# IvanIZ/BenchPush

Hardware: AMD Instinct MI355X
Metric: env-steps/sec at N=4096 envs (ship-ice-v0), 1/2/4/8 MI355X (higher is better)
Workload: dtype f64

## Files before the change

benchpush_amd/build.py:

```python
import os
import subprocess

_HERE = os.path.dirname(os.path.abspath(__file__))
CSRC = os.path.join(_HERE, "csrc")
LIB_PATH = os.path.join(_HERE, "libbenchpush_hip.so")
SOURCES = ["bp_capi.hip"]


def _headers():
    import glob
    return sorted(glob.glob(os.path.join(CSRC, "*.hpp"))) + [os.path.join(_HERE, "..", "include", "benchpush_amd.h")]

HIPCC_FLAGS = ["--offload-arch=gfx950", "-O3", "-ffp-contract=off", "-fno-fast-math", "-fPIC", "-shared", "-std=c++17",
               "-Wno-unused-value"]


def needs_build():
    if not os.path.exists(LIB_PATH):
        return True
    t = os.path.getmtime(LIB_PATH)
    for p in [os.path.join(CSRC, f) for f in SOURCES] + _headers():
        if os.path.exists(p) and os.path.getmtime(p) > t:
            return True
    return False


def build_hip(force=False, verbose=False):
    if not force and not needs_build():
        return LIB_PATH
    hipcc = os.environ.get("HIPCC", "/opt/rocm/bin/hipcc")
    if not os.path.exists(hipcc):
        hipcc = "hipcc"
    cmd = [hipcc] + HIPCC_FLAGS + ["-o", LIB_PATH] + [os.path.join(CSRC, s) for s in SOURCES]
    if verbose:
        print(" ".join(cmd))
    subprocess.check_call(cmd, cwd=CSRC)
    return LIB_PATH


DBG_LIB_PATH = os.path.join(_HERE, "libbenchpush_hip_dbgpaths.so")


def build_debug_paths(force=False, verbose=False):
    if not force and os.path.exists(DBG_LIB_PATH):
        t = os.path.getmtime(DBG_LIB_PATH)
        if all(os.path.getmtime(p) <= t for p in [os.path.join(CSRC, f) for f in SOURCES] + _headers() if os.path.exists(p)):
            return DBG_LIB_PATH
    hipcc = os.environ.get("HIPCC", "/opt/rocm/bin/hipcc")
    if not os.path.exists(hipcc):
        hipcc = "hipcc"
    cmd = [hipcc] + HIPCC_FLAGS + ["-DBP_DEBUG_PATHS=1", "-o", DBG_LIB_PATH] + [os.path.join(CSRC, s) for s in SOURCES]
    if verbose:
        print(" ".join(cmd))
    subprocess.check_call(cmd, cwd=CSRC)
    return DBG_LIB_PATH


PROF_LIB_PATH = os.path.join(_HERE, "libbenchpush_hip_prof.so")


def build_prof(force=False, verbose=False):
    if not force and os.path.exists(PROF_LIB_PATH):
        t = os.path.getmtime(PROF_LIB_PATH)
        if all(os.path.getmtime(p) <= t for p in [os.path.join(CSRC, f) for f in SOURCES] + _headers() if os.path.exists(p)):
            return PROF_LIB_PATH
    hipcc = os.environ.get("HIPCC", "/opt/rocm/bin/hipcc")
    if not os.path.exists(hipcc):
        hipcc = "hipcc"
    cmd = [hipcc] + HIPCC_FLAGS + ["-DBP_PROF=1", "-o", PROF_LIB_PATH] + [os.path.join(CSRC, s) for s in SOURCES]
    if verbose:
        print(" ".join(cmd))
    subprocess.check_call(cmd, cwd=CSRC)
    return PROF_LIB_PATH


if __name__ == "__main__":
    print(build_hip(force=True, verbose=True))
    print(build_debug_paths(force=True, verbose=True))
    print(build_prof(force=True, verbose=True))
```

benchpush_amd/csrc/bp_physics.hpp:

```cpp
#pragma once
#include "bp_device.hpp"
#include <type_traits>

#ifdef BP_PROF
#define PROF_DECL unsigned long long _pt = __builtin_amdgcn_s_memtime();
#define PROF_ACC(slot) { unsigned long long _n = __builtin_amdgcn_s_memtime(); if (lane_id() == 0) L.prof[slot] += _n - _pt; _pt = _n; }
#define PROF_CNT(slot, v) { const unsigned long long _v = (unsigned long long)(v); if (lane_id() == 0) L.prof[slot] += _v; }
#define PROF_MAX(slot, v) { const unsigned long long _v = (unsigned long long)(v); if (lane_id() == 0 && _v > L.prof[slot]) L.prof[slot] = _v; }
#define PROF_PARAM , unsigned long long &_pt
#define PROF_ARG , _pt
#else
#define PROF_DECL
#define PROF_ACC(slot)
#define PROF_CNT(slot, v)
#define PROF_MAX(slot, v)
#define PROF_PARAM
#define PROF_ARG
#endif


#define BP_UNLIKELY(x) __builtin_expect(!!(x), 0)
#define BP_UNLIKELY2(x) __builtin_expect(!!(x), 0)
#ifdef BP_DEBUG_PATHS
#define BP_DBGP(bit) ((P.dbg_paths & (bit)) != 0)
#define BP_TRACE_ON(D) ((D).dbg != nullptr)
#else
#define BP_DBGP(bit) false
#define BP_TRACE_ON(D) false
#endif
#ifndef BP_BOUND_GROUPS
#define BP_BOUND_GROUPS 3
#endif
#ifndef BP_MANIFOLD_LANES
#define BP_MANIFOLD_LANES 2
#endif
#include "bp_contact.hpp"

struct EnvCtx {
    int nb;
    const int *nv;
    const d2 *lv, *ln;
    const double4 *mass;
    const double4 *prop;
    const int *kind;
    d2 *pxy, *rot, *wv, *wn, *pv;
    double *ang;
    double4 *bb, *fat;
    unsigned short *adj;
    unsigned char *adjn;
    unsigned long long *hint;
};

template <typename T> __device__ __forceinline__ T &gE(T *const base, const int idx) { return *(T *)((char *)base + (size_t)((unsigned)idx * (unsigned)sizeof(T))); }

struct LdsCtx {
    d2 *sv, *sw, *sb;
    d2 *ag;
    d2 *sp;
    unsigned char *slot_of;
    unsigned *mvs;
    unsigned short *owner;
    unsigned short *colmask;
    d2 *tf;
    unsigned short *mv;
    unsigned *mvo;
    unsigned short *sbody;
    unsigned char *rf;
// ... 323 lines not shown
        const bool hitQ = (xh & 1) != 0;
        const unsigned h = sd ? ((unsigned)(xh >> 1) << 8) | (unsigned)eia : ((unsigned)eia << 8) | (unsigned)(xh >> 1);
        const bool any = hit || hitQ, two = hit && hitQ;
        PROF_CNT(54, (unsigned long long)__popcll(ballot(sd == 0 && hit && !hitQ)) | ((unsigned long long)__popcll(ballot(sd == 0 && !hit && hitQ)) << 32))
        PROF_CNT(55, __popcll(ballot(sd == 0 && two)))
        PROF_ACC(10)
        const bool flagonly = (cw & (1u << 19)) != 0;
        if (ballot(any && flagonly)) S.wall_flag = 1;
        const bool del = any && !flagonly;
        const unsigned long long dm = ballot(del && sd == 0);
        const int drank = popc_below(dm, lane & ~1);
        const int ndel = __popcll(dm);
        const unsigned keyv = (e.x << 16) | (e.x >> 16);
        lds_sync();
        for (int dbase = 0; dbase < ndel; dbase += BP_MBOX) {
            if (del && drank >= dbase && drank < dbase + BP_MBOX) {
                d2 *mb = L.mbox + (drank - dbase) * 6;
                if (sd == 0) {
                    mb[0] = n;
                    if (hit) { mb[1] = p1; mb[2] = p2; mb[5].x = __hiloint2double((int)h, two ? 2 : 1); }
                } else {
                    if (!hitQ) { mb[1] = p1; mb[2] = p2; mb[5].x = __hiloint2double((int)h, 1); }
                    mb[3] = two ? p1 : mk2(0, 0); mb[4] = two ? p2 : mk2(0, 0);
                    mb[5].y = __hiloint2double(two ? (int)h : 0, 0);
                }
            }
            lds_sync();
            arbiters_take(E, L, A, S, dm, dbase, keyv, now);
            lds_sync();
        }
    }
}

template <int KIND, bool DAMP = false>
__device__ __forceinline__ void substep(const DevParams &P, const EnvCtx &E, const LdsCtx &L, ArbReg &A, SubState &S,
                                        const double dt, const int ship_rules)
{
    const int lane = lane_id();
    constexpr int VL = (KIND == BP_ENV_BOX) ? 4 : (KIND == BP_ENV_MAZE) ? 8 : BP_MAXV;
    constexpr bool ML2 = (BP_MANIFOLD_LANES == 2) && KIND != BP_ENV_BOX;
    if (KIND == BP_ENV_BOX) { S.nev = 0; S.evmask = 0ull; }
    S.stamp += 1u;
    const unsigned now = S.stamp;
    const double prev_dt = S.curr_dt;
    S.curr_dt = dt;
    if (A.key != ARB_FREE_KEY && A.stamp == now - 1u) A.state = ARB_NORMAL;
    PROF_DECL
    PROF_CNT(16, S.nmv)

    for (int k0 = 0; k0 < S.nmv; k0 += 64) {
        const int k = k0 + lane;
        double rad = 0.0;
        double4 fatb; fatb.x = fatb.y = -BP_INF; fatb.z = fatb.w = BP_INF;
        if (k < S.nmv) {
            const int i = L.mv[k];
            const int sl = L.slot_of[i];
            d2 v = mk2(0.0, 0.0), w2 = mk2(0.0, 0.0), vb = mk2(0.0, 0.0);
            if (sl != 255) { v = L.sv[sl]; w2 = L.sw[sl]; vb = L.sb[sl]; }
            d2 p = gE(E.pxy, i);
            if (sl != 255) p = L.sp[sl];
            const double a = gE(E.ang, i);
            d2 r = gE(E.rot, i);
            const double4 ms = gE(E.mass, i);
            rad = gE(E.prop, i).x;
            fatb = gE(E.fat, i);
            L.rf[lane] = (unsigned char)gE(E.nv, i);
            p.x = p.x + (v.x + vb.x) * dt;
            p.y = p.y + (v.y + vb.y) * dt;
            const double a2 = a + (w2.x + w2.y) * dt;
            if (a2 != a) { double sn, cs; bp_sincos(a2, sn, cs); r = mk2(cs, sn); }
            gE(E.pxy, i) = p; gE(E.ang, i) = a2; gE(E.rot, i) = r;
            if (i == 0) { L.ag[0] = mk2(a2, 0.0); L.ag[1] = r; }
            if (sl != 255) { L.sb[sl] = mk2(0.0, 0.0); L.sw[sl].y = 0.0; L.sp[sl] = p; }
// ... 40 lines not shown
            nbb.x = key_f64(bbk[lane * 4 + 0]) - rad; nbb.y = key_f64(bbk[lane * 4 + 2]) - rad;
            nbb.z = key_f64(bbk[lane * 4 + 1]) + rad; nbb.w = key_f64(bbk[lane * 4 + 3]) + rad;
            gE(E.bb, i) = nbb;
            leftfat = !(nbb.x >= fatb.x && nbb.y >= fatb.y && nbb.z <= fatb.z && nbb.w <= fatb.w);
        }
        PROF_ACC(0)
        unsigned long long rm = ballot(leftfat);
        if (BP_UNLIKELY(rm != 0)) { S.cc_ok = 0; __syncthreads(); }
        while (BP_UNLIKELY(rm != 0)) {
            const int kk = __ffsll((long long)rm) - 1;
            rm &= rm - 1;
            refresh_body(P, E, L.mv[k0 + kk], S.err);
            PROF_CNT(17, 1)
        }
        PROF_ACC(1)
    }
    __syncthreads();
    PROF_ACC(35)

    int kmax = S.cc_kmax;
    if (!S.cc_ok) {
        kmax = 0;
        for (int k0 = 0; k0 < S.nmv; k0 += 64) {
            const int k = k0 + lane;
            const int cnt = (k < S.nmv) ? (int)gE(E.adjn, L.mv[k]) : 0;
            int m = 0;
            for (int bit = 16; bit >= 1; bit >>= 1) { if (ballot(cnt >= (m | bit))) m |= bit; }
            kmax = max(kmax, m);
        }
        S.cc_kmax = kmax;
    }
    const int ncand_slots = S.nmv * kmax;
    for (int base = 0; base < ncand_slots; base += 64) {
        int i, j, s, nA_h, nB_h;
        bool valid, flagonly;
        unsigned long long hw;
        const bool cached = S.cc_ok && base == 0 && !BP_DBGP(1);
        if (cached) {
            const unsigned long long c = L.cc[lane];
            hw = L.cc_hw[lane];
            static_assert(2 * BP_CC_IDX_BITS == 28, "cc word layout: i | j << BP_CC_IDX_BITS | slot << 28 ...");
            i = (int)(c & ((1u << BP_CC_IDX_BITS) - 1u)); j = (int)((c >> BP_CC_IDX_BITS) & ((1u << BP_CC_IDX_BITS) - 1u)); s = (int)((c >> 28) & 31u);
            nA_h = (int)((c >> 33) & 31u); nB_h = (int)((c >> 38) & 31u);
            valid = ((c >> 43) & 1u) != 0; flagonly = ((c >> 44) & 1u) != 0;
        } else {
            const int idx = base + lane;
            const int k = idx / kmax;
            s = idx - k * kmax;
            const bool inlist = k < S.nmv;
            i = inlist ? (int)L.mv[k] : 0;
            const int sc = min(s, BP_KADJ - 1);
            const int adjn_i = gE(E.adjn, i);
            j = gE(E.adj, i * BP_KADJ + sc) < E.nb ? (int)gE(E.adj, i * BP_KADJ + sc) : 0;
            hw = gE(E.hint, i * BP_KADJ + sc);
            valid = inlist && (s < adjn_i);
            if (valid && L.mvs[j] == now && j < i) valid = false;
            const int ki = gE(E.kind, i), kj = gE(E.kind, j);
            const double mi = gE(E.mass, i).x, mj = gE(E.mass, j).x;
            nA_h = gE(E.nv, min(i, j)); nB_h = gE(E.nv, max(i, j));
            flagonly = false;
            if (valid) {
                if (kind_group(ki) != 0 && kind_group(ki) == kind_group(kj)) valid = false;
                else if (mi == 0.0 && mj == 0.0) {
                    const int ci = kind_ctype(ki), cj = kind_ctype(kj);
                    flagonly = (ci == 1 && cj == 3) || (ci == 3 && cj == 1);
                    valid = flagonly;
                }
            }
            s = min(s, 31);
            if (base == 0) {
                L.cc[lane] = (unsigned long long)(unsigned)i | ((unsigned long long)(unsigned)j << BP_CC_IDX_BITS) | ((unsigned long long)(unsigned)s << 28) |
                             ((unsigned long long)(unsigned)nA_h << 33) | ((unsigned long long)(unsigned)nB_h << 38) |
                             ((unsigned long long)(valid ? 1u : 0u) << 43) | ((unsigned long long)(flagonly ? 1u : 0u) << 44);
                L.cc_hw[lane] = hw;
            }
        }
        const int sc = min(s, BP_KADJ - 1);
        const int sa = min(i, j), sb = max(i, j);
        const double4 bbi = gE(E.bb, i);
        const double4 bbj = gE(E.bb, j);
        const double radA = gE(E.prop, sa).x, radB = gE(E.prop, sb).x;
        const double rsum = radA + radB;
        const int hA = HW_PLANE_A(hw) < BP_MAXV ? HW_PLANE_A(hw) : 0, hB = HW_PLANE_B(hw) < BP_MAXV ? HW_PLANE_B(hw) : 0;
        const int cnA = HW_NV_A(hw), cnB = HW_NV_B(hw);
        const int jA0 = HW_VERT_A(hw) < BP_MAXV ? HW_VERT_A(hw) : 0, jB0 = HW_VERT_B(hw) < BP_MAXV ? HW_VERT_B(hw) : 0;
        const int jAm = (jA0 == 0) ? max(min(cnB, BP_MAXV) - 1, 0) : jA0 - 1, jAp = (jA0 + 1 >= cnB) ? 0 : jA0 + 1;
        const int jBm = (jB0 == 0) ? max(min(cnA, BP_MAXV) - 1, 0) : jB0 - 1, jBp = (jB0 + 1 >= cnA) ? 0 : jB0 + 1;
        const d2 fnA = gE(E.wn, sa * BP_MAXV + hA), fpA = gE(E.wv, sa * BP_MAXV + hA);
        const d2 fnB = gE(E.wn, sb * BP_MAXV + hB), fpB = gE(E.wv, sb * BP_MAXV + hB);
        const d2 vAm = gE(E.wv, sb * BP_MAXV + jAm), vA0 = gE(E.wv, sb * BP_MAXV + jA0), vAp = gE(E.wv, sb * BP_MAXV + jAp);
        const d2 vBm = gE(E.wv, sa * BP_MAXV + jBm), vB0 = gE(E.wv, sa * BP_MAXV + jB0), vBp = gE(E.wv, sa * BP_MAXV + jBp);
        if (valid) valid = bb_overlap(bbi, bbj);
        PROF_ACC(27)
        PROF_CNT(24, 1)
        PROF_CNT(36, __popcll(ballot(valid)))
        if (ballot(valid) == 0) { PROF_ACC(2) continue; }
        const bool evA = valid && (hw & HW_HAS_A) && ((hw & HW_BOTH) || !(hw & HW_PRIM_B));
        const bool evB = valid && (hw & HW_HAS_B) && ((hw & HW_BOTH) || (hw & HW_PRIM_B));
        double sepAc = -BP_INF, sepBc = -BP_INF;
        int jAc = jA0, jBc = jB0;
        const double cA = vdot(fnA, fpA), cB = vdot(fnB, fpB);
        bool qryA = evA, qryB = evB;
        {
            const double dm = vdot(fnA, vAm), d0 = vdot(fnA, vA0), dp = vdot(fnA, vAp);
            if (evA && cnB == nB_h && cnB >= 2 && d0 + BP_SUPPORT_MARGIN <= dm && d0 + BP_SUPPORT_MARGIN <= dp && !BP_DBGP(4)) { sepAc = (d0 - cA) + 0.0; qryA = false; }
        }
        {
            const double dm = vdot(fnB, vBm), d0 = vdot(fnB, vB0), dp = vdot(fnB, vBp);
            if (evB && cnA == nA_h && cnA >= 2 && d0 + BP_SUPPORT_MARGIN <= dm && d0 + BP_SUPPORT_MARGIN <= dp && !BP_DBGP(4)) { sepBc = (d0 - cB) + 0.0; qryB = false; }
        }
        {
            const unsigned long long mqA = ballot(qryA), mqB = ballot(qryB);
            const int nqA = __popcll(mqA), nq1 = nqA + __popcll(mqB);
            PROF_CNT(37, nq1)
            if (BP_UNLIKELY(nq1)) {
                const int slA = popc_below(mqA, lane), slB = nqA + popc_below(mqB, lane);
                for (int q0 = 0; q0 < nq1; q0 += BP_QCAP) {
                    const bool inA = qryA && slA >= q0 && slA < q0 + BP_QCAP, inB = qryB && slB >= q0 && slB < q0 + BP_QCAP;
                    if (inA) { L.q_dir[slA - q0] = fnA; L.q_meta[slA - q0] = (unsigned)sb | ((unsigned)nB_h << 16); }
                    if (inB) { L.q_dir[slB - q0] = fnB; L.q_meta[slB - q0] = (unsigned)sa | ((unsigned)nA_h << 16); }
                    lds_sync();
                    support_queries<VL>(E, L, min(nq1 - q0, BP_QCAP));
                    lds_sync();
                    if (inA) { sepAc = (L.r_val[slA - q0] - cA) + 0.0; jAc = (int)L.r_idx[slA - q0]; }
                    if (inB) { sepBc = (L.r_val[slB - q0] - cB) + 0.0; jBc = (int)L.r_idx[slB - q0]; }
                    lds_sync();
                }
            }
        }
        if (valid && (sepAc > rsum || sepBc > rsum)) {
            valid = false;
            if (hw & HW_BOTH) {
                const unsigned long long nh = (hw & ~(HW_BOTH | HW_PRIM_B)) | ((sepAc > rsum) ? 0ull : HW_PRIM_B);
                gE(E.hint, i * BP_KADJ + s) = nh;
                if (base == 0) L.cc_hw[lane] = nh;
            }
        }
        const unsigned long long cm = ballot(valid);
        PROF_ACC(28)
        PROF_CNT(18, __popcll(cm))
        if (cm == 0) continue;
        PROF_CNT(25, 1)
        const int nc = __popcll(cm);
        const int myr = popc_below(cm, lane);
        const int nA_l = valid ? nA_h : 0, nB_l = valid ? nB_h : 0;
        if (valid) {
            uint4 pa;
            pa.x = (unsigned)sa | ((unsigned)sb << 16);
            pa.y = (unsigned)nA_l | (evA ? 0x80u : 0u) | ((unsigned)nB_l << 8) | ((unsigned)hA << 16) | ((unsigned)jAc << 24);
            pa.z = (unsigned)sb | ((unsigned)sa << 16);
            pa.w = (unsigned)nB_l | (evB ? 0x80u : 0u) | ((unsigned)nA_l << 8) | ((unsigned)hB << 16) | ((unsigned)jBc << 24);
            L.pt_a[myr] = pa;
            L.pt_thr[myr] = mk2(sepAc, sepBc);
            L.res_smA[myr] = evA ? f64_key(sepAc) : 0ull; L.res_iA[myr] = evA ? ((unsigned)hA << 8) | (unsigned)jAc : 0xFFFFFFFFu;
            L.res_smB[myr] = evB ? f64_key(sepBc) : 0ull; L.res_iB[myr] = evB ? ((unsigned)hB << 8) | (unsigned)jBc : 0xFFFFFFFFu;
            static_assert(BP_CC_IDX_BITS + 5 <= 19 && BP_KADJ <= 32, "candidate lane's word: i | slot << BP_CC_IDX_BITS | flagonly << 19 | lane << 20");
            if (ML2) L.res_jA[myr] = (unsigned)i | ((unsigned)s << BP_CC_IDX_BITS) | (flagonly ? 1u << 19 : 0u) | ((unsigned)lane << 20);
        }
        lds_sync();
        {
            int nq = 0, g0 = 0;
            const uint2 *const pts = (const uint2 *)L.pt_a;
            const double *const pts_thr = (const double *)L.pt_thr;
            auto round_addr = [&](const uint2 e, int &pbody, int &qbody, int &np, int &nqv, int &hX, bool &evX, int &jc, int &jm, int &jp) {
                pbody = (int)(e.x & 0xFFFFu); qbody = (int)(e.x >> 16);
                np = (int)(e.y & 0x7Fu); evX = (e.y & 0x80u) != 0; nqv = (int)((e.y >> 8) & 0xFFu);
                hX = (int)((e.y >> 16) & 0xFFu); jc = (int)(e.y >> 24);
                jm = (jc == 0) ? max(nqv, 1) - 1 : jc - 1; jp = (jc + 1 >= nqv) ? 0 : jc + 1;
            };
            int rr_start = nc;
            {
                constexpr int GW = (BP_BOUND_GROUPS == 3 && KIND != BP_ENV_BOX) ? BP_MAXV + 1 : 32, IPR = 64 / GW;
                static_assert(GW >= BP_MAXV && IPR * GW <= 64, "a lane group holds every plane of a side");
                const int g = lane / GW, f = lane - g * GW;
                const int ipr = BP_DBGP(16) ? 1 : IPR;
                bool fits = !BP_DBGP(2);
                for (int r0 = 0; r0 < nc && fits; r0 += ipr) {
                    const bool on0 = g < ipr && 2 * r0 + g < 2 * nc, on1 = g < ipr && 2 * r0 + ipr + g < 2 * nc;
                    const int ta = on0 ? 2 * r0 + g : 2 * r0, tb = on1 ? 2 * r0 + ipr + g : 2 * r0;
                    const uint2 e0 = pts[ta], e1 = pts[tb];
                    const double th0 = pts_thr[ta], th1 = pts_thr[tb];
                    int pb0, qb0, np0, nqv0, hX0, jc0, jm0, jp0, pb1, qb1, np1, nqv1, hX1, jc1, jm1, jp1; bool ev0, ev1;
                    round_addr(e0, pb0, qb0, np0, nqv0, hX0, ev0, jc0, jm0, jp0);
                    round_addr(e1, pb1, qb1, np1, nqv1, hX1, ev1, jc1, jm1, jp1);
                    const int fc0 = (f < np0) ? f : 0, fc1 = (f < np1) ? f : 0;
                    const d2 fn0 = gE(E.wn, pb0 * BP_MAXV + fc0), fp0 = gE(E.wv, pb0 * BP_MAXV + fc0), vb0 = gE(E.wv, qb0 * BP_MAXV + jc0), vm0 = gE(E.wv, qb0 * BP_MAXV + jm0), vp0 = gE(E.wv, qb0 * BP_MAXV + jp0);
                    const d2 fn1 = gE(E.wn, pb1 * BP_MAXV + fc1), fp1 = gE(E.wv, pb1 * BP_MAXV + fc1), vb1 = gE(E.wv, qb1 * BP_MAXV + jc1), vm1 = gE(E.wv, qb1 * BP_MAXV + jm1), vp1 = gE(E.wv, qb1 * BP_MAXV + jp1);
                    {
                        const bool pv = on0 && (f < np0) && !(ev0 && f == hX0);
                        const double c = vdot(fn0, fp0);
// ... 18 lines not shown
                        if (surv && sl < BP_QCAP) {
                            L.q_dir[sl] = fn1; L.q_meta[sl] = (unsigned)qb1 | ((unsigned)nqv1 << 16);
                            L.q_aux[sl] = (unsigned)(tb >> 1) | ((unsigned)(tb & 1) << 8) | ((unsigned)f << 16);
                            L.q_c[sl] = c;
                        }
                        nq += __popcll(sm);
                    }
                    PROF_CNT(49, 1)
                    fits = nq <= BP_QCAP;
                }
                if (!fits) { nq = 0; rr_start = 0; }
                lds_sync();
            }
            const int side = lane >> 5, f = lane & 31;
            for (int rr = rr_start; rr <= nc; rr++) {
                if (nq > 0 && (rr == nc || nq + 64 > BP_QCAP)) {
                    PROF_ACC(29)
                    support_queries<VL>(E, L, nq);
                    lds_sync();
                    PROF_CNT(26, 1)
                    PROF_CNT(38, nq)
                    for (int s0 = 0; s0 < nq; s0 += 64) {
                        const int sl = s0 + lane;
                        if (sl < nq) {
                            const unsigned aux = L.q_aux[sl];
                            const int r = (int)(aux & 0xFFu);
                            const double sp = (L.r_val[sl] - L.q_c[sl]) + 0.0;
                            const unsigned long long key = f64_key(sp);
                            L.q_c[sl] = __builtin_bit_cast(double, key);
                            atomicMax((aux & 0x100u) ? &L.res_smB[r] : &L.res_smA[r], key);
                        }
                    }
                    lds_sync();
                    if (valid && myr >= g0 && myr < rr) {
                        if (evA && f64_key(sepAc) != L.res_smA[myr]) L.res_iA[myr] = 0xFFFFFFFFu;
                        if (evB && f64_key(sepBc) != L.res_smB[myr]) L.res_iB[myr] = 0xFFFFFFFFu;
                    }
                    lds_sync();
                    for (int s0 = 0; s0 < nq; s0 += 64) {
                        const int sl = s0 + lane;
                        if (sl < nq) {
                            const unsigned aux = L.q_aux[sl];
                            const int r = (int)(aux & 0xFFu);
                            const unsigned long long key = __builtin_bit_cast(unsigned long long, L.q_c[sl]);
                            if (key == ((aux & 0x100u) ? L.res_smB[r] : L.res_smA[r])) atomicMin((aux & 0x100u) ? &L.res_iB[r] : &L.res_iA[r], ((aux >> 16) << 8) | L.r_idx[sl]);
                        }
                    }
                    lds_sync();
                    nq = 0; g0 = rr;
                    PROF_ACC(30)
                }
                if (rr == nc) break;
                const uint2 e = pts[2 * rr + side];
                const double th = pts_thr[2 * rr + side];
                int pbody, qbody, np, nqv, hX, jc, jm, jp; bool evX;
                round_addr(e, pbody, qbody, np, nqv, hX, evX, jc, jm, jp);
                const bool pv = (f < np) && !(evX && f == hX);
                const int fc = (f < np) ? f : 0;
                const d2 fn = gE(E.wn, pbody * BP_MAXV + fc), fp = gE(E.wv, pbody * BP_MAXV + fc);
                const d2 vb = gE(E.wv, qbody * BP_MAXV + jc), vm = gE(E.wv, qbody * BP_MAXV + jm), vp = gE(E.wv, qbody * BP_MAXV + jp);
                const double c = vdot(fn, fp);
                const double bound = (fmin(vdot(fn, vb), fmin(vdot(fn, vm), vdot(fn, vp))) - c) + 0.0;
                const bool surv = pv && (!evX || bound >= th);
                const unsigned long long sm = ballot(surv);
                if (surv) {
                    const int sl = nq + popc_below(sm, lane);
                    L.q_dir[sl] = fn; L.q_meta[sl] = (unsigned)qbody | ((unsigned)nqv << 16);
// ... 426 lines not shown
                if (AB) {
                    const d2 vb1 = vadd(vba, vmul(vperp(r1), wa2.y));
                    const d2 vb2 = vadd(vbb, vmul(vperp(r2), wb2.y));
                    const double vbn = vdot(vsub(vb2, vb1), n);
                    const double jbn = (bias - vbn) * nMass;
                    jBias = fmax(jbnOld + jbn, 0.0);
                }
                const double jn = -(bounce + vrn) * nMass;
                const double jnOld = c ? A.jn1 : A.jn0;
                const double jnAcc = fmax(jnOld + jn, 0.0);
                const double jtMax = A.u * jnAcc;
                const double jt = -vrt * tMass;
                const double jtOld = c ? A.jt1 : A.jt0;
                const double jtAcc = fclampd(jtOld + jt, -jtMax, jtMax);
                if (c) { jBias1 = jBias; A.jn1 = jnAcc; A.jt1 = jtAcc; }
                else   { jBias0 = jBias; A.jn0 = jnAcc; A.jt0 = jtAcc; }
                if (AB) {
                    const double djb = jBias - jbnOld;
                    chg += __builtin_fabs(djb);
                    const d2 jb = vmul(n, djb);
                    const d2 jbneg = vneg(jb);
                    vba = vadd(vba, vmul(jbneg, A.ma));
                    wa2.y += A.ia * vcross(r1, jbneg);
                    vbb = vadd(vbb, vmul(jb, A.mb));
                    wb2.y += A.ib * vcross(r2, jb);
                }
                const double djn = jnAcc - jnOld, djt = jtAcc - jtOld;
                chg += __builtin_fabs(djn); chg += __builtin_fabs(djt);
                const d2 j = vrotate(n, mk2(djn, djt));
                apply_contact_impulses(A, c, va, wa2.x, vb, wb2.x, j);
            }
        }
    };
    if (!AB && KIND != BP_ENV_BOX && (lvlmask & (lvlmask - 1u)) == 0u && lvlmask != 0u) {
        d2 va = mk2(0.0, 0.0), vb = va, wa2 = va, wb2 = va, vba = va, vbb = va;
        if (solve) gather(va, vb, wa2, wb2, vba, vbb);
        bool nz = false;
        if (solve && A.ma == 0.0) nz = is_negzero(va.x) || is_negzero(va.y) || is_negzero(wa2.x) || (AB && (is_negzero(wa2.y) || is_negzero(vba.x) || is_negzero(vba.y)));
        if (solve && A.mb == 0.0) nz = nz || is_negzero(vb.x) || is_negzero(vb.y) || is_negzero(wb2.x) || (AB && (is_negzero(wb2.y) || is_negzero(vbb.x) || is_negzero(vbb.y)));
        if (!ballot(nz)) {
            for (int it = 0; it < P.iterations; it++) {
                PROF_CNT(42, 1)
                PROF_CNT(43, 1)
                double chg = 0.0;
                if (solve) contacts(va, vb, wa2, wb2, vba, vbb, chg);
                if (BP_UNLIKELY2(!ballot(solve && chg != 0.0))) break;
            }
            if (solve) scatter(va, vb, wa2, wb2, vba, vbb);
            lds_sync();
            return;
        }
    }
    for (int it = 0; it < P.iterations; it++) {
        PROF_CNT(42, 1)
        double chg = 0.0;
        for (unsigned lm = lvlmask; lm; lm &= lm - 1u) {
            const int lvl = __ffs((int)lm) - 1;
            PROF_CNT(43, 1)
            PROF_CNT(44, ballot(solve && A.level == lvl && A.count > 1) ? 1 : 0)
            if (solve && A.level == lvl) {
                d2 va, vb, wa2, wb2, vba, vbb;
                gather(va, vb, wa2, wb2, vba, vbb);
                contacts(va, vb, wa2, wb2, vba, vbb, chg);
                scatter(va, vb, wa2, wb2, vba, vbb);
            }
            lds_sync();
        }
        if (BP_UNLIKELY2(!ballot(solve && chg != 0.0))) break;
    }
    };
    if (any_bias && !mirrored) iterate(std::true_type{}); else iterate(std::false_type{});
    PROF_ACC(8)
    {
        const bool shiparb = active && ba == 0;
        const unsigned long long sm = ballot(shiparb);
        S.ship_post = (unsigned)__popcll(sm);
        S.ship_contacts = (unsigned)__popcll(sm) + (unsigned)__popcll(ballot(shiparb && A.count > 1));
        if (sm) {
            S.n_post += (unsigned)__popcll(sm);
            S.n_contact += (unsigned)__popcll(sm) + (unsigned)__popcll(ballot(shiparb && A.count > 1));
            S.n_first += (unsigned)__popcll(ballot(shiparb && A.state == ARB_FIRST));
            const bool ws = shiparb && warm;
            const unsigned long long wsm = ballot(ws);
            if (wsm) {
                const double e_first = readlane_f64(A.e, __ffsll((long long)wsm) - 1);
                double eCoef;
                if (!ballot(ws && A.e != e_first)) {
                    if (e_first != S.ecoef_e) { S.ecoef_e = e_first; S.ecoef = (1 - e_first) / (1 + e_first); }
                    eCoef = S.ecoef;
// ... 94 lines not shown
```

benchpush_amd/csrc/bp_capi.hip:

```cpp
#include <hip/hip_runtime.h>

#include <cstdio>
#include <cstdlib>
#include <algorithm>
#include <cstring>
#include <map>
#include <mutex>
#include <string>
#include <vector>

#include <fcntl.h>
#include <sys/file.h>
#include <sys/stat.h>
#include <unistd.h>

#include "bp_host_bd.hpp"
#include "bp_boxdelivery.hpp"
#include "bp_policy.hpp"
#include "bp_render.hpp"
#include "bp_state.hpp"
#include "bp_swath.hpp"
#include "bp_lattice.hpp"
#include "bp_track.hpp"
#include "bp_rrt.hpp"
// ... 197 lines not shown

int32_t bp_abi_version(void) { return BP_ABI_VERSION; }
int32_t bp_sizeof_config(void) { return (int32_t)sizeof(bp_config); }

const char *bp_last_error(const bp_handle *h) { return h ? h->err.c_str() : "null handle"; }

int bp_create(const bp_config *cfg, int32_t num_envs, int64_t env_id_offset, int32_t device, bp_handle **out)
{
    if (!cfg || !out || num_envs <= 0) return BP_EINVAL;
    *out = nullptr;
    int ndev = 0;
    if (hipGetDeviceCount(&ndev) != hipSuccess || ndev <= 0 || device < 0 || device >= ndev) return BP_ENODEVICE;
    if (!(cfg->damping_pow >= 0.0) || cfg->damping_pow > 1.0) return BP_EINVAL;
    if (cfg->num_ship_verts < 3 || cfg->num_ship_verts > BP_MAX_SHIP_VERTS) return BP_EINVAL;
    if (cfg->steps <= 0 || cfg->iterations <= 0 || cfg->persistence <= 0) return BP_EINVAL;
    if (cfg->env_kind != BP_ENV_SHIP_ICE && cfg->env_kind != BP_ENV_MAZE) return BP_EINVAL;
    if (cfg->env_kind == BP_ENV_MAZE && (cfg->num_wheels < 0 || cfg->num_wheels > BP_MAX_WHEELS)) return BP_EINVAL;
    if (cfg->random_start && cfg->env_kind != BP_ENV_SHIP_ICE) return BP_EINVAL;
    bp_handle *h = new bp_handle();
    h->cfg = *cfg;
    h->num_envs = num_envs;
    h->env_offset = env_id_offset;
    h->device = device;
    h->resettle = (cfg->env_kind == BP_ENV_SHIP_ICE && cfg->random_start != 0);
    DevGuard _dg(device);
    if (!_dg.ok) { delete h; return BP_ENODEVICE; }
    memset(&h->D, 0, sizeof(h->D));
    DevParams &P = h->P;
    memset(&P, 0, sizeof(P));
    P.dt_sub = cfg->dt / cfg->steps;
    P.steps = cfg->steps; P.iterations = cfg->iterations; P.persistence = cfg->persistence; P.settle_steps = cfg->settle_steps;
    if (const char *evp = getenv("BP_DEBUG_PATHS")) P.dbg_paths = atoi(evp);
    P.bias_lanes = getenv("BP_BIAS_LANES") ? (atoi(getenv("BP_BIAS_LANES")) != 0) : 1;
    P.damping_pow = cfg->damping_pow; P.bias_coef = cfg->bias_coef; P.slop = cfg->slop;
    P.target_speed = cfg->target_speed; P.max_yaw_rate = cfg->max_yaw_rate;
    P.map_w = cfg->map_w; P.map_h = cfg->map_h; P.goal_y = cfg->goal_y; P.m_to_pix = cfg->m_to_pix;
    P.beta = cfg->beta; P.boundary_penalty = cfg->boundary_penalty; P.terminal_reward = cfg->terminal_reward;
    P.local_w = cfg->local_w; P.local_h = cfg->local_h; P.vshift = cfg->vshift; P.obs_range = cfg->obs_range;
    P.skin = 0.06;
    P.env_kind = cfg->env_kind;
    P.nkin = (cfg->env_kind == BP_ENV_MAZE) ? 1 + cfg->num_wheels : 1;
    P.goal_x = cfg->goal_x; P.goal_reach = cfg->goal_reach; P.k_increment = cfg->k_increment;
    P.num_envs = num_envs; P.env_offset = env_id_offset;
    P.random_start = (cfg->env_kind == BP_ENV_SHIP_ICE) ? cfg->random_start : 0;
    P.start_x_range = cfg->start_x_range; P.start_seed = cfg->start_seed; P.ship_mass = cfg->ship_mass;
    P.num_ship_verts = cfg->num_ship_verts;
    memcpy(P.ship_verts, cfg->ship_verts, sizeof(P.ship_verts));
    memcpy(P.ship_head, cfg->ship_head, sizeof(P.ship_head));
    memcpy(P.ship_tail, cfg->ship_tail, sizeof(P.ship_tail));
    const double grid = 1.0 / cfg->m_to_pix;
    P.grid_w = (int)(cfg->map_w / grid);
    P.grid_h = (int)(cfg->map_h / grid);
    P.obs_h = (int)(cfg->local_h * cfg->m_to_pix);
    P.obs_w = (int)(cfg->local_w * cfg->m_to_pix);
    if ((P.obs_h * P.obs_w) % 4 != 0) { delete h; return BP_EINVAL; }
    if (cfg->env_kind == BP_ENV_MAZE) {
        const int infl = (P.obs_w > P.obs_h ? P.obs_w : P.obs_h) / 2;
        const int nwords = ((P.obs_h + infl) * (P.obs_w + infl) + 31) / 32;
        h->obs_lds_bytes = (size_t)4 * (nwords + ((nwords + 1) & ~1)) + sizeof(double) * 2 * MZ_MAXBOX * 4;
        if (hipFuncSetAttribute((const void *)k_observe_maze, hipFuncAttributeMaxDynamicSharedMemorySize, (int)h->obs_lds_bytes) != hipSuccess) { delete h; return BP_EHIP; }
    } else {
        if (P.obs_h % 2 != 0 || P.obs_w % 2 != 0 || P.obs_w / 2 > OBS_THREADS_SHIP) { delete h; return BP_EINVAL; }
        h->obs_lds_bytes = (size_t)((P.obs_h * P.obs_w + 15) & ~15) + (size_t)((P.obs_h + 15) & ~15) + sizeof(double) * 2 * OBS_CHUNK * BP_MAXV;
        if (hipFuncSetAttribute((const void *)k_observe, hipFuncAttributeMaxDynamicSharedMemorySize, (int)h->obs_lds_bytes) != hipSuccess) { delete h; return BP_EHIP; }
    }
    *out = h;
// ... 2038 lines not shown
```

benchpush_amd/csrc/bp_device.hpp:

```cpp
#pragma once
#include <hip/hip_runtime.h>
#include <stdint.h>

#include "../../include/benchpush_amd.h"

#define BP_KADJ 24
#define BP_ACAP 64

typedef double2 d2;

enum { BODY_DYNAMIC = 0, BODY_KINEMATIC = 1, BODY_STATIC = 2 };
__device__ __forceinline__ int kind_ctype(int k) { return k & 0xFF; }
__device__ __forceinline__ int kind_group(int k) { return (k >> 8) & 0xFF; }
__device__ __forceinline__ int kind_btype(int k) { return (k >> 16) & 3; }
enum { ARB_FIRST = 0, ARB_NORMAL = 1, ARB_IGNORE = 2, ARB_CACHED = 3 };
#define ARB_FREE_KEY 0xFFFFFFFFu

struct DevParams {
    double dt_sub;
    int steps, iterations, persistence, settle_steps;
    double damping_pow, bias_coef, slop, target_speed, max_yaw_rate, map_w, map_h, goal_y, m_to_pix;
    double beta, boundary_penalty, terminal_reward, local_w, local_h, vshift, obs_range;
    double goal_x, goal_reach, k_increment;
    int env_kind;
    int nkin;
    double skin;
    int nbcap, mvcap, num_envs, num_trials, num_ship_verts;
    long long env_offset;
    double ship_verts[BP_MAX_SHIP_VERTS][2];
    double ship_head[2], ship_tail[2];
    int obs_h, obs_w, grid_h, grid_w;
    int sq_chunk, sq_levels, sq_cap;
    int sq_cls;
    unsigned sq_ymask;
    int sq_dynprio;
    int sq_parts, sq_part;
    int sq_floor;
    int sq_lrpt, sq_bw, sq_hyst;
    int sq_hold;
    int sq_mode;
    int sq_image;
    unsigned sq_img_lds;
    unsigned sq_img_stride;
    int sq_debug;
    int bias_lanes;
    int dbg_paths;
    int pair_mode, pair_solo;
    int pp_max_keys, pp_max_slots, pp_max_mv, pp_max_act, pp_max_work;
    int pp_snake, pp_heavy_only;
    int pp_rate;
    int random_start;
    double start_x_range, ship_mass;
    unsigned long long start_seed;
};

struct DevPtrs {
    const int *sc_nb;
    const int *sc_nv;
    const d2 *sc_lv;
    const d2 *sc_ln;
    const double4 *sc_mass;
    const double4 *sc_pose;
    const double4 *sc_prop;
    const int *sc_kind;
    const double *dist_map;
    const unsigned char *wall_map;
    const double *goal_raw;
    const double *maze_obs_map;
    int *e_trial, *e_episode, *e_nb, *e_err;
    int *e_flags;
    double *e_prevdist;
    unsigned *e_stamp;
    double *e_currdt, *e_total_work, *e_ke, *e_imp;
    unsigned *e_cnt;
    unsigned *e_cost;
    const int *order;
    int *sq_items;
    int *sq_ctr;
    unsigned *sq_carry;
    unsigned char *sq_moved;
    unsigned char *sq_img;
    int *sq_done;
    int *sq_lev;
    unsigned *sq_thr;
    int *sq_sub;
    int *sq_pairstat;
// ... 257 lines not shown
```

Measured before the change: 300,300.

## Split cached candidate pairs across two lanes, one per collision side

Adds a candidate-evaluation path that gives each cached candidate pair two lanes, one per body side. Each lane computes the face-support separation, support query and plane record for its own side. The path is used when the candidate cache is valid and there are at most 32 candidate slots. It is meant to halve per-lane serial work on ship/box-like scenes where few candidates fill a wavefront. The later validity check is rewritten to read the per-side records, and the path adds extra lane-pair exchanges and a new code path that must match the single-lane layout.

```diff
diff --git a/benchpush_amd/build.py b/benchpush_amd/build.py
--- a/benchpush_amd/build.py
+++ b/benchpush_amd/build.py
@@ -39,6 +39,7 @@
 
 
 DBG_LIB_PATH = os.path.join(_HERE, "libbenchpush_hip_dbgpaths.so")
+TWIN_FLAGS = ["-DBP_CAND_LANES=2"]
 
 
 def build_debug_paths(force=False, verbose=False):
@@ -49,7 +50,7 @@
     hipcc = os.environ.get("HIPCC", "/opt/rocm/bin/hipcc")
     if not os.path.exists(hipcc):
         hipcc = "hipcc"
-    cmd = [hipcc] + HIPCC_FLAGS + ["-DBP_DEBUG_PATHS=1", "-o", DBG_LIB_PATH] + [os.path.join(CSRC, s) for s in SOURCES]
+    cmd = [hipcc] + HIPCC_FLAGS + ["-DBP_DEBUG_PATHS=1"] + TWIN_FLAGS + ["-o", DBG_LIB_PATH] + [os.path.join(CSRC, s) for s in SOURCES]
     if verbose:
         print(" ".join(cmd))
     subprocess.check_call(cmd, cwd=CSRC)
@@ -67,7 +68,7 @@
     hipcc = os.environ.get("HIPCC", "/opt/rocm/bin/hipcc")
     if not os.path.exists(hipcc):
         hipcc = "hipcc"
-    cmd = [hipcc] + HIPCC_FLAGS + ["-DBP_PROF=1", "-o", PROF_LIB_PATH] + [os.path.join(CSRC, s) for s in SOURCES]
+    cmd = [hipcc] + HIPCC_FLAGS + ["-DBP_PROF=1"] + TWIN_FLAGS + ["-o", PROF_LIB_PATH] + [os.path.join(CSRC, s) for s in SOURCES]
     if verbose:
         print(" ".join(cmd))
     subprocess.check_call(cmd, cwd=CSRC)
diff --git a/benchpush_amd/csrc/bp_physics.hpp b/benchpush_amd/csrc/bp_physics.hpp
--- a/benchpush_amd/csrc/bp_physics.hpp
+++ b/benchpush_amd/csrc/bp_physics.hpp
@@ -33,6 +33,9 @@
 #endif
 #ifndef BP_MANIFOLD_LANES
 #define BP_MANIFOLD_LANES 2
+#endif
+#ifndef BP_CAND_LANES
+#define BP_CAND_LANES 2
 #endif
 #include "bp_contact.hpp"
 
@@ -422,6 +425,97 @@
     }
 }
 
+template <int VL>
+__device__ __forceinline__ int candidates_side_lanes(const DevParams &P, const EnvCtx &E, const LdsCtx &L PROF_PARAM)
+{
+    const int lane = lane_id();
+    const int q = lane >> 1, sd = lane & 1;
+    const unsigned long long cw = L.cc[q];
+    const unsigned long long hw = L.cc_hw[q];
+    const int i = (int)(cw & ((1u << BP_CC_IDX_BITS) - 1u)), j = (int)((cw >> BP_CC_IDX_BITS) & ((1u << BP_CC_IDX_BITS) - 1u)), s = (int)((cw >> 28) & 31u);
+    const int nA_h = (int)((cw >> 33) & 31u), nB_h = (int)((cw >> 38) & 31u);
+    bool valid = ((cw >> 43) & 1u) != 0;
+    const bool flagonly = ((cw >> 44) & 1u) != 0;
+    PROF_CNT(22, 1)
+    const int sa = min(i, j), sb = max(i, j);
+    const int bO = sd ? sb : sa, bQ = sd ? sa : sb;
+    const int nQ_h = sd ? nA_h : nB_h;
+    const double4 bbi = gE(E.bb, i);
+    const double4 bbj = gE(E.bb, j);
+    const double radA = gE(E.prop, sa).x, radB = gE(E.prop, sb).x;
+    const double rsum = radA + radB;
+    const unsigned hf = (unsigned)hw >> (sd ? 5 : 0);
+    const int hO = (int)(hf & 31u) < BP_MAXV ? (int)(hf & 31u) : 0;
+    const int cnQ = sd ? HW_NV_A(hw) : HW_NV_B(hw);
+    const int j0 = (int)((hf >> 10) & 31u) < BP_MAXV ? (int)((hf >> 10) & 31u) : 0;
+    const int jm = (j0 == 0) ? max(min(cnQ, BP_MAXV) - 1, 0) : j0 - 1, jp = (j0 + 1 >= cnQ) ? 0 : j0 + 1;
+    const d2 fn = gE(E.wn, bO * BP_MAXV + hO), fp = gE(E.wv, bO * BP_MAXV + hO);
+    const d2 vm = gE(E.wv, bQ * BP_MAXV + jm), v0 = gE(E.wv, bQ * BP_MAXV + j0), vp = gE(E.wv, bQ * BP_MAXV + jp);
+    if (valid) valid = bb_overlap(bbi, bbj);
+    PROF_ACC(27)
+    PROF_CNT(24, 1)
+    PROF_CNT(36, __popcll(ballot(valid && sd == 0)))
+    if (ballot(valid) == 0) { PROF_ACC(2) return 0; }
+    const bool has = ((hw >> (32 + sd)) & 1ull) != 0;
+    const bool primO = (int)((hw >> 34) & 1ull) == sd;
+    const bool ev = valid && has && ((hw & HW_BOTH) || primO);
+    double sep = -BP_INF;
+    int jc = j0;
+    const double c = vdot(fn, fp);
+    bool qry = ev;
+    {
+        const double dm = vdot(fn, vm), d0 = vdot(fn, v0), dp = vdot(fn, vp);
+        if (ev && cnQ == nQ_h && cnQ >= 2 && d0 + BP_SUPPORT_MARGIN <= dm && d0 + BP_SUPPORT_MARGIN <= dp && !BP_DBGP(4)) { sep = (d0 - c) + 0.0; qry = false; }
+    }
+    {
+        const unsigned long long mq = ballot(qry);
+        const int nq1 = __popcll(mq);
+        PROF_CNT(37, nq1)
+        PROF_CNT(52, (unsigned long long)__popcll(mq & 0x5555555555555555ull) << 32)
+        PROF_CNT(55, (unsigned long long)__popcll(mq & 0xAAAAAAAAAAAAAAAAull) << 32)
+        if (BP_UNLIKELY(nq1)) {
+            const int sl = popc_below(mq, lane);
+            for (int q0 = 0; q0 < nq1; q0 += BP_QCAP) {
+                const bool in = qry && sl >= q0 && sl < q0 + BP_QCAP;
+                if (in) { L.q_dir[sl - q0] = fn; L.q_meta[sl - q0] = (unsigned)bQ | ((unsigned)nQ_h << 16); }
+                lds_sync();
+                support_queries<VL>(E, L, min(nq1 - q0, BP_QCAP));
+                lds_sync();
+                if (in) { sep = (L.r_val[sl - q0] - c) + 0.0; jc = (int)L.r_idx[sl - q0]; }
+                lds_sync();
+            }
+        }
+    }
+    const int clrO = (valid && sep > rsum) ? 1 : 0;
+    const int clrQ = mate_i32(clrO);
+    if (clrO | clrQ) {
+        valid = false;
+        if (sd == 0 && (hw & HW_BOTH)) {
+            const unsigned long long nh = (hw & ~(HW_BOTH | HW_PRIM_B)) | (clrO ? 0ull : HW_PRIM_B);
+            gE(E.hint, i * BP_KADJ + s) = nh;
+            L.cc_hw[q] = nh;
+        }
+    }
+    const unsigned long long cm = ballot(valid && sd == 0);
+    PROF_ACC(28)
+    PROF_CNT(18, __popcll(cm))
+    if (cm == 0) return 0;
+    PROF_CNT(25, 1)
+    if (valid) {
+        const int myr = popc_below(cm, lane & ~1);
+        const int nO_h = sd ? nB_h : nA_h;
+        uint2 pe;
+        pe.x = (unsigned)bO | ((unsigned)bQ << 16);
+        pe.y = (unsigned)nO_h | (ev ? 0x80u : 0u) | ((unsigned)nQ_h << 8) | ((unsigned)hO << 16) | ((unsigned)jc << 24);
+        ((uint2 *)L.pt_a)[2 * myr + sd] = pe;
+        ((double *)L.pt_thr)[2 * myr + sd] = sep;
+        L.res_smA[sd * 64 + myr] = ev ? f64_key(sep) : 0ull;
+        L.res_iA[sd * 64 + myr] = ev ? ((unsigned)hO << 8) | (unsigned)jc : 0xFFFFFFFFu;
+        if (sd == 0) L.res_jA[myr] = (unsigned)i | ((unsigned)s << BP_CC_IDX_BITS) | (flagonly ? 1u << 19 : 0u) | ((unsigned)q << 20);
+    }
+    return __popcll(cm);
+}
+
 template <int KIND, bool DAMP = false>
 __device__ __forceinline__ void substep(const DevParams &P, const EnvCtx &E, const LdsCtx &L, ArbReg &A, SubState &S,
                                         const double dt, const int ship_rules)
@@ -429,6 +523,7 @@
     const int lane = lane_id();
     constexpr int VL = (KIND == BP_ENV_BOX) ? 4 : (KIND == BP_ENV_MAZE) ? 8 : BP_MAXV;
     constexpr bool ML2 = (BP_MANIFOLD_LANES == 2) && KIND != BP_ENV_BOX;
+    constexpr bool CL2 = (BP_CAND_LANES == 2) && ML2 && KIND != BP_ENV_MAZE;
     if (KIND == BP_ENV_BOX) { S.nev = 0; S.evmask = 0ull; }
     S.stamp += 1u;
     const unsigned now = S.stamp;
@@ -535,9 +630,18 @@
     }
     const int ncand_slots = S.nmv * kmax;
     for (int base = 0; base < ncand_slots; base += 64) {
-        int i, j, s, nA_h, nB_h;
-        bool valid, flagonly;
-        unsigned long long hw;
+        int i = 0, j = 0, s = 0, nA_h = 0, nB_h = 0;
+        bool valid = false, flagonly = false;
+        unsigned long long hw = 0ull;
+        int nc = 0, myr = 0, sa = 0, sb = 0, nA_l = 0, nB_l = 0;
+        double radA = 0.0, radB = 0.0, rsum = 0.0, sepAc = -BP_INF, sepBc = -BP_INF;
+        bool evA = false, evB = false;
+        if (CL2 && base == 0 && ncand_slots <= 32 && S.cc_ok && !BP_DBGP(128 | 32 | 1)) {
+            nc = candidates_side_lanes<VL>(P, E, L PROF_ARG);
+            if (nc == 0) continue;
+        } else {
+        if (KIND != BP_ENV_BOX) { PROF_CNT(22, 1ull << 32) }
+        if (CL2 && base == 0 && ncand_slots <= 32 && !S.cc_ok) { PROF_CNT(50, 1ull << 32) }
         const bool cached = S.cc_ok && base == 0 && !BP_DBGP(1);
         if (cached) {
             const unsigned long long c = L.cc[lane];
@@ -579,11 +683,11 @@
             }
         }
         const int sc = min(s, BP_KADJ - 1);
-        const int sa = min(i, j), sb = max(i, j);
+        sa = min(i, j); sb = max(i, j);
         const double4 bbi = gE(E.bb, i);
         const double4 bbj = gE(E.bb, j);
-        const double radA = gE(E.prop, sa).x, radB = gE(E.prop, sb).x;
-        const double rsum = radA + radB;
+        radA = gE(E.prop, sa).x; radB = gE(E.prop, sb).x;
+        rsum = radA + radB;
         const int hA = HW_PLANE_A(hw) < BP_MAXV ? HW_PLANE_A(hw) : 0, hB = HW_PLANE_B(hw) < BP_MAXV ? HW_PLANE_B(hw) : 0;
         const int cnA = HW_NV_A(hw), cnB = HW_NV_B(hw);
         const int jA0 = HW_VERT_A(hw) < BP_MAXV ? HW_VERT_A(hw) : 0, jB0 = HW_VERT_B(hw) < BP_MAXV ? HW_VERT_B(hw) : 0;
@@ -598,9 +702,8 @@
         PROF_CNT(24, 1)
         PROF_CNT(36, __popcll(ballot(valid)))
         if (ballot(valid) == 0) { PROF_ACC(2) continue; }
-        const bool evA = valid && (hw & HW_HAS_A) && ((hw & HW_BOTH) || !(hw & HW_PRIM_B));
-        const bool evB = valid && (hw & HW_HAS_B) && ((hw & HW_BOTH) || (hw & HW_PRIM_B));
-        double sepAc = -BP_INF, sepBc = -BP_INF;
+        evA = valid && (hw & HW_HAS_A) && ((hw & HW_BOTH) || !(hw & HW_PRIM_B));
+        evB = valid && (hw & HW_HAS_B) && ((hw & HW_BOTH) || (hw & HW_PRIM_B));
         int jAc = jA0, jBc = jB0;
         const double cA = vdot(fnA, fpA), cB = vdot(fnB, fpB);
         bool qryA = evA, qryB = evB;
@@ -644,9 +747,9 @@
         PROF_CNT(18, __popcll(cm))
         if (cm == 0) continue;
         PROF_CNT(25, 1)
-        const int nc = __popcll(cm);
-        const int myr = popc_below(cm, lane);
-        const int nA_l = valid ? nA_h : 0, nB_l = valid ? nB_h : 0;
+        nc = __popcll(cm);
+        myr = popc_below(cm, lane);
+        nA_l = valid ? nA_h : 0; nB_l = valid ? nB_h : 0;
         if (valid) {
             uint4 pa;
             pa.x = (unsigned)sa | ((unsigned)sb << 16);
@@ -659,6 +762,7 @@
             L.res_smB[myr] = evB ? f64_key(sepBc) : 0ull; L.res_iB[myr] = evB ? ((unsigned)hB << 8) | (unsigned)jBc : 0xFFFFFFFFu;
             static_assert(BP_CC_IDX_BITS + 5 <= 19 && BP_KADJ <= 32, "candidate lane's word: i | slot << BP_CC_IDX_BITS | flagonly << 19 | lane << 20");
             if (ML2) L.res_jA[myr] = (unsigned)i | ((unsigned)s << BP_CC_IDX_BITS) | (flagonly ? 1u << 19 : 0u) | ((unsigned)lane << 20);
+        }
         }
         lds_sync();
         {
@@ -743,7 +847,12 @@
                         }
                     }
                     lds_sync();
-                    if (valid && myr >= g0 && myr < rr) {
+                    if (CL2) {
+                        for (int b0 = g0; b0 < rr; b0 += 32) {
+                            const int br = b0 + (lane >> 1), bt = 2 * br + (lane & 1), bk = (lane & 1) * 64 + br;
+                            if (br < rr && (pts[bt].y & 0x80u) && f64_key(pts_thr[bt]) != L.res_smA[bk]) L.res_iA[bk] = 0xFFFFFFFFu;
+                        }
+                    } else if (valid && myr >= g0 && myr < rr) {
                         if (evA && f64_key(sepAc) != L.res_smA[myr]) L.res_iA[myr] = 0xFFFFFFFFu;
                         if (evB && f64_key(sepBc) != L.res_smB[myr]) L.res_iB[myr] = 0xFFFFFFFFu;
                     }
```

Measured after the change: 302,300, median of 6. About the same (+0.7%).

## Add kinematic-side fast path for ship-ice contact solver level

Applied to the files above, without the earlier changes.

When every arbiter in the first constraint level has a kinematic or static A body (zero mass and inertia), the solver now caches A's contact-point velocities once and updates only the B side each iteration. This skips the per-iteration gather and scatter of the A body and the A-side impulse writes. Odd values (NaN, inf, denormals, huge normals) disable the path, and a large-change check falls back to reapplying the A side exactly. It adds code complexity and a new environment flag, which is on by default.

```diff
diff --git a/benchpush_amd/csrc/bp_capi.hip b/benchpush_amd/csrc/bp_capi.hip
--- a/benchpush_amd/csrc/bp_capi.hip
+++ b/benchpush_amd/csrc/bp_capi.hip
@@ -253,6 +253,7 @@
     P.steps = cfg->steps; P.iterations = cfg->iterations; P.persistence = cfg->persistence; P.settle_steps = cfg->settle_steps;
     if (const char *evp = getenv("BP_DEBUG_PATHS")) P.dbg_paths = atoi(evp);
     P.bias_lanes = getenv("BP_BIAS_LANES") ? (atoi(getenv("BP_BIAS_LANES")) != 0) : 1;
+    P.kin_side = getenv("BP_KIN_SIDE") ? (atoi(getenv("BP_KIN_SIDE")) != 0) : 1;
     P.damping_pow = cfg->damping_pow; P.bias_coef = cfg->bias_coef; P.slop = cfg->slop;
     P.target_speed = cfg->target_speed; P.max_yaw_rate = cfg->max_yaw_rate;
     P.map_w = cfg->map_w; P.map_h = cfg->map_h; P.goal_y = cfg->goal_y; P.m_to_pix = cfg->m_to_pix;
diff --git a/benchpush_amd/csrc/bp_device.hpp b/benchpush_amd/csrc/bp_device.hpp
--- a/benchpush_amd/csrc/bp_device.hpp
+++ b/benchpush_amd/csrc/bp_device.hpp
@@ -52,6 +52,7 @@
     int random_start;
     double start_x_range, ship_mass;
     unsigned long long start_seed;
+    int kin_side;
 };
 
 struct DevPtrs {
diff --git a/benchpush_amd/csrc/bp_physics.hpp b/benchpush_amd/csrc/bp_physics.hpp
--- a/benchpush_amd/csrc/bp_physics.hpp
+++ b/benchpush_amd/csrc/bp_physics.hpp
@@ -1236,6 +1236,41 @@
             }
         }
     };
+    constexpr bool KIN = !AB && KIND == BP_ENV_SHIP_ICE;
+    constexpr double KIN_BOUND = 0x1p300;
+    auto kin_over = [](const double chg) { return (unsigned)__double2hiint(chg) >= 0x52B00000u; };
+    auto kballot = [](const bool p) { return __builtin_amdgcn_ballot_w64(p); };
+    constexpr int KIN_ODD = 0x001 | 0x002 | 0x004 | 0x020 | 0x200;
+    auto kcontact = [&](const int c, const d2 v1, d2 &vb, double &wb, double &chg, d2 &j) {
+        const d2 n = A.n;
+        const d2 r2 = c ? A.r2_1 : A.r2_0;
+        const double nMass = c ? nMass1 : nMass0, tMass = c ? tMass1 : tMass0;
+        const double bounce = c ? bounce1 : bounce0;
+        const d2 v2 = vadd(vb, vmul(vperp(r2), wb));
+        const d2 vr = vsub(v2, v1);
+        const double vrn = vdot(vr, n);
+        const double vrt = vdot(vr, vperp(n));
+        const double jn = -(bounce + vrn) * nMass;
+        const double jnOld = c ? A.jn1 : A.jn0;
+        const double jnAcc = fmax(jnOld + jn, 0.0);
+        const double jtMax = A.u * jnAcc;
+        const double jt = -vrt * tMass;
+        const double jtOld = c ? A.jt1 : A.jt0;
+        const double jtAcc = fclampd(jtOld + jt, -jtMax, jtMax);
+        if (c) { A.jn1 = jnAcc; A.jt1 = jtAcc; }
+        else   { A.jn0 = jnAcc; A.jt0 = jtAcc; }
+        const double djn = jnAcc - jnOld, djt = jtAcc - jtOld;
+        chg += __builtin_fabs(djn); chg += __builtin_fabs(djt);
+        j = vrotate(n, mk2(djn, djt));
+        vb = vadd(vb, vmul(j, A.mb));
+        wb += A.ib * vcross(r2, j);
+    };
+    auto kside_a = [&](const int c, d2 &va, double &wa, const d2 j) {
+        const d2 r1 = c ? A.r1_1 : A.r1_0;
+        const d2 jn = vneg(j);
+        va = vadd(va, vmul(jn, A.ma));
+        wa += A.ia * vcross(r1, jn);
+    };
     if (!AB && KIND != BP_ENV_BOX && (lvlmask & (lvlmask - 1u)) == 0u && lvlmask != 0u) {
         d2 va = mk2(0.0, 0.0), vb = va, wa2 = va, wb2 = va, vba = va, vbb = va;
         if (solve) gather(va, vb, wa2, wb2, vba, vbb);
@@ -1246,6 +1281,7 @@
             for (int it = 0; it < P.iterations; it++) {
                 PROF_CNT(42, 1)
                 PROF_CNT(43, 1)
+                PROF_CNT(22, 1ull << 21)
                 double chg = 0.0;
                 if (solve) contacts(va, vb, wa2, wb2, vba, vbb, chg);
                 if (BP_UNLIKELY2(!ballot(solve && chg != 0.0))) break;
@@ -1255,10 +1291,49 @@
             return;
         }
     }
+    unsigned kinmask = 0;
+    d2 v1k0 = mk2(0.0, 0.0), v1k1 = v1k0;
+    if (KIN && P.kin_side != 0 && !BP_DBGP(128) && lvlmask != 0u) {
+        const int lvl0 = __ffs((int)lvlmask) - 1;
+        if (!ballot(solve && A.level == lvl0 && (A.ma != 0.0 || A.ia != 0.0))) kinmask = 1u << lvl0;
+        if (kinmask) {
+            const bool mine = solve && ((kinmask >> (A.level & 31)) & 1u) != 0u;
+            d2 va = mk2(0.0, 0.0);
+            double wa = 0.0;
+            if (mine) { va = *gvA; wa = *gwA; }
+            const double big = fmax(fmax(__builtin_fabs(A.n.x), __builtin_fabs(A.n.y)), fmax(__builtin_fabs(A.r1_0.x), __builtin_fabs(A.r1_0.y)));
+            const bool odd = mine && (__builtin_amdgcn_class(va.x, KIN_ODD) || __builtin_amdgcn_class(va.y, KIN_ODD) || __builtin_amdgcn_class(wa, KIN_ODD) || !(big < KIN_BOUND));
+            if (BP_UNLIKELY(ballot(odd))) kinmask = 0;
+            v1k0 = vadd(va, vmul(vperp(A.r1_0), wa));
+            v1k1 = vadd(va, vmul(vperp(A.r1_1), wa));
+        }
+    }
+    const bool kin_in = KIN && kinmask != 0u && solve && ((kinmask >> (A.level & 31)) & 1u) != 0u;
+    const unsigned restmask = (KIN && kinmask != 0u) ? (lvlmask & ~kinmask) : lvlmask;
     for (int it = 0; it < P.iterations; it++) {
         PROF_CNT(42, 1)
         double chg = 0.0;
-        for (unsigned lm = lvlmask; lm; lm &= lm - 1u) {
+        if (KIN && kinmask != 0u) {
+            PROF_CNT(43, 1)
+            PROF_CNT(44, ballot(kin_in && A.count > 1) ? 1 : 0)
+            PROF_CNT(22, 1)
+            if (kin_in) {
+                d2 vb = *gvB, j;
+                double wb = *gwB;
+                kcontact(0, v1k0, vb, wb, chg, j);
+                if (A.count > 1) {
+                    if (BP_UNLIKELY(kballot(kin_over(chg)))) {
+                        d2 va = *gvA;
+                        double wa = *gwA;
+                        kside_a(0, va, wa, j);
+                        kcontact(1, vadd(va, vmul(vperp(A.r1_1), wa)), vb, wb, chg, j);
+                    } else kcontact(1, v1k1, vb, wb, chg, j);
+                }
+                *svB = vb; *swB = wb;
+            }
+            lds_sync();
+        }
+        for (unsigned lm = restmask; lm; lm &= lm - 1u) {
             const int lvl = __ffs((int)lm) - 1;
             PROF_CNT(43, 1)
             PROF_CNT(44, ballot(solve && A.level == lvl && A.count > 1) ? 1 : 0)
```

Result: no change. 298,900 before, 298,700 after (-0.1%).
